# ska-telescope/ska-sdp-idg-bench

Hardware: AMD Instinct MI355X
Metric: Mvisibilities/s (gridder & degridder) at 1/2/4/8 GPUs; % HBM roofline (higher is better)
Workload: dtype f32 phase/accumulate, f16x2-split MFMA operands

## Files before the change

### ska-sdp-idg-bench_amd/csrc/hip/kernels/gridder_mi355x.hip.cpp

```cpp
#include <hip/hip_runtime.h>

#include <cstdlib>
#include <string>

#include "../util.hpp"
#include "device.hpp"
#include "fft.hpp"
#include "lib-hip.hpp"
#include "mfma.hpp"

#ifndef IDG_GRID_PT
#define IDG_GRID_PT 4
#endif
#ifndef IDG_GRID_WAVES
#define IDG_GRID_WAVES 4
#endif
#ifndef IDG_GRID_WAVES_GENERAL
#define IDG_GRID_WAVES_GENERAL 4
#endif
#ifndef IDG_GRID_FUSED_GENERAL
#define IDG_GRID_FUSED_GENERAL 1
#endif
#ifndef IDG_GRID_BSCALE
#define IDG_GRID_BSCALE 12
#endif
#ifndef IDG_GRID_NT_FILL
#define IDG_GRID_NT_FILL 0
#endif
#ifndef IDG_GRID_NW
#define IDG_GRID_NW 8
#endif

namespace idg_mi355x {

namespace {

__device__ __forceinline__ void mac4(float *a, const float4 &va,
                                     const float4 &vb, float cs, float sn) {
  a[0] = fma_(va.x, cs, a[0]); a[0] = fma_(-va.y, sn, a[0]);
  a[1] = fma_(va.x, sn, a[1]); a[1] = fma_(va.y, cs, a[1]);
  a[2] = fma_(va.z, cs, a[2]); a[2] = fma_(-va.w, sn, a[2]);
  a[3] = fma_(va.z, sn, a[3]); a[3] = fma_(va.w, cs, a[3]);
  a[4] = fma_(vb.x, cs, a[4]); a[4] = fma_(-vb.y, sn, a[4]);
  a[5] = fma_(vb.x, sn, a[5]); a[5] = fma_(vb.y, cs, a[5]);
  a[6] = fma_(vb.z, cs, a[6]); a[6] = fma_(-vb.w, sn, a[6]);
  a[7] = fma_(vb.z, sn, a[7]); a[7] = fma_(vb.w, cs, a[7]);
}

template <int NP, int CB>
__device__ __forceinline__ void timestep_general(
    const float (&l)[NP], const float (&m)[NP], const float (&n)[NP],
    const float (&poff)[NP], float (&acc)[NP][8],
    const idg::UVWCoordinate<float> c, const float4 *__restrict__ vrow,
    const float *__restrict__ wavenumbers, int C) {
  float pidx[NP];
#pragma unroll
  for (int i = 0; i < NP; ++i)
    pidx[i] = fma_(c.w, n[i], fma_(c.u, l[i], c.v * m[i]));
  for (int cb = 0; cb < C; cb += CB) {
    const int ce = min(cb + CB, C);
    const float k0 = wavenumbers[cb];
    float A[NP], R[NP];
#pragma unroll
    for (int i = 0; i < NP; ++i) {
      A[i] = fma_(-pidx[i], k0, poff[i]);
      R[i] = revolutions(A[i]);
    }
    float k = k0;
    float4 va = vrow[2 * cb], vb = vrow[2 * cb + 1];
    for (int ch = cb; ch < ce; ++ch) {
      const int nx = min(ch + 1, C - 1);
      const float kn = wavenumbers[nx];
      const float4 van = vrow[2 * nx], vbn = vrow[2 * nx + 1];
#pragma unroll
      for (int i = 0; i < NP; ++i) {
        const float ph = fma_(-pidx[i], k, poff[i]);
        const float r = fma_(ph - A[i], kInv2PiHi, R[i]);
        float sn, cs;
        sincos_rev(r, &sn, &cs);
        mac4(acc[i], va, vb, cs, sn);
      }
      k = kn;
      va = van;
      vb = vbn;
    }
  }
}

template <int NB, int CB>
__device__ __forceinline__ void timestep_mirror(
    const float (&l)[2 * NB], const float (&m)[2 * NB],
    const float (&poff)[2 * NB], float (&acc)[2 * NB][8],
    const idg::UVWCoordinate<float> c, const float4 *__restrict__ vrow,
    const float *__restrict__ wavenumbers, int C) {
  float pidx[NB];
#pragma unroll
  for (int i = 0; i < NB; ++i) pidx[i] = fma_(c.u, l[i], c.v * m[i]);
  for (int cb = 0; cb < C; cb += CB) {
    const int ce = min(cb + CB, C);
    const float k0 = wavenumbers[cb];
    float A[NB], R[NB];
#pragma unroll
    for (int i = 0; i < NB; ++i) {
      A[i] = fma_(-pidx[i], k0, poff[i]);
      R[i] = revolutions(A[i]);
    }
    float k = k0;
    float4 va = vrow[2 * cb], vb = vrow[2 * cb + 1];
    for (int ch = cb; ch < ce; ++ch) {
      const int nx = min(ch + 1, C - 1);
      const float kn = wavenumbers[nx];
      const float4 van = vrow[2 * nx], vbn = vrow[2 * nx + 1];
#pragma unroll
      for (int i = 0; i < NB; ++i) {
        const float ph = fma_(-pidx[i], k, poff[i]);
        const float r = fma_(ph - A[i], kInv2PiHi, R[i]);
        float sn, cs;
        sincos_rev(r, &sn, &cs);
        mac4(acc[i], va, vb, cs, sn);
        mac4(acc[NB + i], va, vb, cs, -sn);
      }
      k = kn;
      va = van;
      vb = vbn;
    }
  }
}

__device__ __forceinline__ void pixel_out(const float (&a)[8], int p, int S,
                                          const SubgridSetup &g,
                                          int nr_stations,
                                          const float *__restrict__ spheroidal,
                                          const float2 *__restrict__ aterms,
                                          float2 (&o)[4]) {
  const int y = p / S, x = p - (p / S) * S;
  idg::cfloat pix[4], a1[4], a2[4];
  for (int q = 0; q < 4; ++q) pix[q] = {a[2 * q], a[2 * q + 1]};
  load_jones(aterm_ptr(aterms, nr_stations, S, g.aterm_index, g.station1, y,
                       x), a1);
  load_jones(aterm_ptr(aterms, nr_stations, S, g.aterm_index, g.station2, y,
                       x), a2);
  idg::apply_aterm_gridder(pix, a1, a2);
  const float sph = spheroidal[p];
#pragma unroll
  for (int q = 0; q < 4; ++q) o[q] = make_float2(pix[q].re * sph, pix[q].im * sph);
}

__device__ __forceinline__ void store_pixel(
    const float (&a)[8], int p, int S, int npix, const SubgridSetup &g,
    int nr_stations, const float *__restrict__ spheroidal,
    const float2 *__restrict__ aterms, float2 *__restrict__ out) {
  float2 o[4];
  pixel_out(a, p, S, g, nr_stations, spheroidal, aterms, o);
#pragma unroll
  for (int q = 0; q < 4; ++q) out[static_cast<size_t>(q) * npix + p] = o[q];
}

template <bool W_TERMS = true>
__device__ __forceinline__ void pixel_geometry(int p, int S, float image_size,
                                               const SubgridSetup &g,
                                               float &l, float &m, float &n,
                                               float &poff) {
  const int y = p / S, x = p - (p / S) * S;
  l = idg::compute_l(x, S, image_size);
  m = idg::compute_m(y, S, image_size);
  if constexpr (W_TERMS) {
    n = idg::compute_n(l, m);
    poff = fma_(g.w_offset, n, fma_(g.u_offset, l, g.v_offset * m));
  } else {
    n = 0.0f;
    poff = fma_(g.u_offset, l, g.v_offset * m);
  }
}


#ifndef IDG_GRID_KSBUF
#define IDG_GRID_KSBUF 32
#endif
constexpr int kKsBuf = IDG_GRID_KSBUF;

template <int AT, int NW>
struct MfmaLds {
  static constexpr int kObufFloats = NW * 16 * AT * 16;
  static constexpr int kBbufWords = kKsBuf * 64 * 8;
  static constexpr int kUvwOff =
      kObufFloats > kBbufWords ? kObufFloats : kBbufWords;
  static constexpr int kRedOff = kUvwOff + 4 * 4 * kKsBuf;
  static constexpr int kSlotOff = kRedOff + 8;
  static constexpr int kSinkOff = kSlotOff + 2;
  static constexpr int kWords = kSinkOff + 64;
  static constexpr int kGeoOff = kWords;
  static constexpr int kWordsGeo = kGeoOff + 64 + 2 * 1024;
};
template <int S_CT, int NW, int AT>
constexpr int general_lds_words() {
  return S_CT == 32 ? MfmaLds<AT, NW>::kWordsGeo : MfmaLds<AT, NW>::kWords;
}

__device__ __forceinline__ void l2_prefetch_dma(const void *src,
                                                const void *lds_dst) {
  const unsigned m0 = __builtin_amdgcn_readfirstlane(static_cast<unsigned>(
      reinterpret_cast<size_t>((const __attribute__((address_space(3))) void *)
                                   lds_dst)));
  unsigned saved;
  asm volatile(
      "s_mov_b32 %0, m0\n\ts_mov_b32 m0, %2\n\ts_nop 0\n\t"
      "global_load_lds_dword %1, off\n\ts_mov_b32 m0, %0"
      : "=&s"(saved)
      : "v"(src), "s"(m0)
      : "memory");
}

template <int S_CT, int PT, int CB, int NW, bool MIRROR, bool FFT = false,
          int PREC = kPrecTail, bool PRESCAN = false, bool OPAQUE_TID = !MIRROR>
__device__ __forceinline__ void grid_mfma(
    const SubgridSetup &g, int S, int npix, float image_size, int C,
    int nr_stations, const idg::UVWCoordinate<float> *__restrict__ uvw,
    const float *__restrict__ wavenumbers,
    const float2 *__restrict__ visibilities,
    const float *__restrict__ spheroidal, const float2 *__restrict__ aterms,
    float2 *__restrict__ out, unsigned *lds, float vmax_pre = 0.0f,
    int pass_lo = 0, int pass_hi = 1 << 30) {
  static_assert(CB % 4 == 0, "anchor blocks hold whole channel quads");
  int tid = threadIdx.x;
  if constexpr (OPAQUE_TID) asm volatile("" : "+v"(tid));
  const int lane = tid & 63, wave = tid >> 6;
  const int grp = lane >> 4, col = lane & 15;
  const int half = MIRROR ? npix / 2 : npix;
  constexpr bool kFused = !MIRROR && IDG_GRID_FUSED_GENERAL;
  constexpr bool kTailAlt = (PREC & kPrecTailAlt) != 0;
  constexpr bool kTailAll = (PREC & kPrecTail) != 0 && !kTailAlt;
  constexpr int AT = kFused ? PT : 2 * PT;
  using Lds = MfmaLds<AT, NW>;
  constexpr bool kGeoLds = kFused && S_CT == 32;
  float *geo = reinterpret_cast<float *>(lds + Lds::kGeoOff);
  const int nt = g.nr_timesteps;
  const int nchq = (C + 3) / 4;
  const int nquads = (nt + 3) / 4;
  const int quads_per_fill = nchq <= kKsBuf ? kKsBuf / nchq : 1;
  const int cq_per_fill = nchq <= kKsBuf ? nchq : kKsBuf;
  unsigned *slots = lds + Lds::kSlotOff;

  float vmax = vmax_pre;
  if (tid < 2) slots[tid] = 0u;
  if constexpr (!PRESCAN) {
    vmax = 0.0f;
    const float4 *v4 = reinterpret_cast<const float4 *>(
        visibilities + g.time_offset * C * 4);
    const int n4 = min(4 * quads_per_fill, nt) * C * 2;
    for (int i = tid; i < n4; i += NW * 64) {
      const float4 q = v4[i];
      vmax = fmaxf(vmax, fmaxf(fmaxf(fabsf(q.x), fabsf(q.y)),
                               fmaxf(fabsf(q.z), fabsf(q.w))));
    }
    for (int off = 32; off > 0; off >>= 1)
      vmax = fmaxf(vmax, __shfl_xor(vmax, off));
    float *red = reinterpret_cast<float *>(lds + Lds::kRedOff);
    if (lane == 0) red[wave] = vmax;
    __syncthreads();
#pragma unroll
    for (int w = 0; w < NW; ++w) vmax = fmaxf(vmax, red[w]);
  }
  constexpr int kBS = IDG_GRID_BSCALE;
  static_assert(kBS >= 0 && kBS <= 14, "a fill may reach 2^15 before it re-splits");
  int e = 0;
  bool have_scale = vmax > 0.0f && vmax <= 3.0e38f;
  if (have_scale) frexpf(vmax, &e);
  float scale = ldexpf(1.0f, kBS - e);
  int fidx = 0;

  const float2 *__restrict__ vsub = visibilities + g.time_offset * C * 4;

  uint4 *bbuf = reinterpret_cast<uint4 *>(lds);
  float *obuf = reinterpret_cast<float *>(lds);
  float4 *tuvw = reinterpret_cast<float4 *>(lds + Lds::kUvwOff);

  constexpr int kPass = NW * 16 * PT;
  for (int gbase = pass_lo; gbase < min(half, pass_hi); gbase += kPass) {
    static_assert(PT % 2 == 0, "phases are packed over tile pairs");
    constexpr int PH = PT / 2;
    floatx2 L2[PH], M2[PH], N2[PH], PG2[PH];
    if constexpr (kGeoLds) {
      static_assert(PT == 8 && NW == 8, "one S = 32 pass: 1,024 pixels");
      for (int p = tid; p < 1024; p += NW * 64) {
        float l, m, n, pg;
        pixel_geometry<true>(p, 32, image_size, g, l, m, n, pg);
        geo[64 + p] = n;
        geo[64 + 1024 + p] = pg;
        if (p < 32) geo[p] = l;
        if (p % 32 == 0) geo[32 + p / 32] = m;
      }
    } else {
#pragma unroll
      for (int i = 0; i < PT; ++i) {
        const int b = min(gbase + (wave * PT + i) * 16 + col, half - 1);
        float l, m, n, pg;
        pixel_geometry<!MIRROR>(b, S, image_size, g, l, m, n, pg);
        L2[i / 2][i % 2] = l;
        M2[i / 2][i % 2] = m;
        N2[i / 2][i % 2] = n;
        PG2[i / 2][i % 2] = pg;
      }
    }
    constexpr int PY = kFused ? 1 : PT;
    floatx4 accx[PT], accy[PY];
#pragma unroll
    for (int i = 0; i < PT; ++i) accx[i] = floatx4{0.0f, 0.0f, 0.0f, 0.0f};
#pragma unroll
    for (int i = 0; i < PY; ++i) accy[i] = floatx4{0.0f, 0.0f, 0.0f, 0.0f};

    constexpr bool kFlush = (PREC & kPrecFlush) != 0;
    static_assert(!kFlush || S_CT == 32,
                  "the master fills the S = 32 output slot in one pass");
    bool flushed = false;
    auto master = [&](int t) {
      return reinterpret_cast<float4 *>(out) +
             ((wave * AT + t) * 32 + grp * 8 + (col & 7));
    };
    auto flush_tile = [&](floatx4 &a, int t, float unsc) {
      const float a0 = a[0], a1 = a[1], a2 = a[2], a3 = a[3];
      const float v0 = (a0 + row_ror8(a0)) * unsc;
      const float v1 = (a1 + row_ror8(a1)) * unsc;
      const float v2 = (a2 + row_ror8(a2)) * unsc;
      const float v3 = (a3 + row_ror8(a3)) * unsc;
      if (col < 8) {
        float4 m = make_float4(0.0f, 0.0f, 0.0f, 0.0f);
        if (flushed) m = *master(t);
        *master(t) = make_float4(m.x + v0, m.y + v1, m.z + v2, m.w + v3);
      }
      a = floatx4{0.0f, 0.0f, 0.0f, 0.0f};
    };

    for (int q0 = 0; q0 < nquads; q0 += quads_per_fill) {
      const int nq = min(quads_per_fill, nquads - q0);
      for (int j0 = 0; j0 < nchq; j0 += cq_per_fill, ++fidx) {
        const int nj = min(cq_per_fill, nchq - j0);
        for (;;) {
        __syncthreads();
        if (tid == 0) slots[(fidx + 1) & 1] = 0u;
        {
          const int bpol = (col & 7) >> 1;
          const int w_c = 2 * bpol + (col & 1);
          const int w_s = 2 * bpol + 1 - (col & 1);
          const float sc_s = (col & 1) ? scale : -scale;
          const float bpart = (col & 8) ? -1.0f : 0.0f;
          const float *vsubf = reinterpret_cast<const float *>(vsub);
          const int nks = nq * nj;
          const bool full = (q0 + nq) * 4 <= nt && 4 * (j0 + nj) <= C;
          const int wv = __builtin_amdgcn_readfirstlane(wave);
          const unsigned off_c = (grp * C * 8 + w_c) * 4u;
          const unsigned off_s = (grp * C * 8 + w_s) * 4u;
          int qq = wv / nj, jj = wv - (wv / nj) * nj;
          float lmax = 0.0f;
#ifdef IDG_DEBUG_SKIPFILL
          for (int ks = fidx > 0 ? nks : wv; ks < nks; ks += NW) {
#else
          for (int ks = wv; ks < nks; ks += NW) {
#endif
            const int t = (q0 + qq) * 4 + grp;
            const int c0 = 4 * (j0 + jj);
            float bc[4], bs[4];
            if (full) {
              const char *blk = reinterpret_cast<const char *>(
                  vsubf + ((q0 + qq) * 4 * C + c0) * 8);
#pragma unroll
              for (int u = 0; u < 4; ++u) {
#if IDG_GRID_NT_FILL
                const __amdgpu_buffer_rsrc_t rsrc =
                    __builtin_amdgcn_make_buffer_rsrc(
                        const_cast<char *>(blk), static_cast<short>(0),
                        0x7ffffff0, 0x00020000);
                const float rc = __builtin_bit_cast(
                    float, __builtin_amdgcn_raw_buffer_load_b32(
                               rsrc, static_cast<int>(off_c), 32 * u, 2));
                const float rs = __builtin_bit_cast(
                    float, __builtin_amdgcn_raw_buffer_load_b32(
                               rsrc, static_cast<int>(off_s), 32 * u, 2));
#else
                const float rc =
                    *reinterpret_cast<const float *>(blk + off_c + 32 * u);
                const float rs =
                    *reinterpret_cast<const float *>(blk + off_s + 32 * u);
#endif
                lmax = fmaxf(lmax, fmaxf(fabsf(rc), fabsf(rs)));
                bc[u] = rc * scale;
                bs[u] = rs * sc_s;
              }
            } else {
#pragma unroll
              for (int u = 0; u < 4; ++u) {
                const bool ok = t < nt && c0 + u < C;
                const int it = ok ? t * C + c0 + u : 0;
                const float rc = ok ? vsubf[it * 8 + w_c] : 0.0f;
                const float rs = ok ? vsubf[it * 8 + w_s] : 0.0f;
                lmax = fmaxf(lmax, fmaxf(fabsf(rc), fabsf(rs)));
                bc[u] = rc * scale;
                bs[u] = rs * sc_s;
              }
            }
            jj += NW;
            while (jj >= nj) {
              jj -= nj;
              ++qq;
            }
            const unsigned xc = split_part(bc[0], bc[1], bpart);
            const unsigned yc = split_part(bc[2], bc[3], bpart);
            const unsigned xs = split_part(bs[0], bs[1], bpart);
            const unsigned ys = split_part(bs[2], bs[3], bpart);
            bbuf[(ks * 64 + lane) * 2] = make_uint4(xc, xc, yc, yc);
            bbuf[(ks * 64 + lane) * 2 + 1] = make_uint4(xs, xs, ys, ys);
          }
          {
            unsigned v = __float_as_uint(lmax);
            v = max(v, (unsigned)__builtin_amdgcn_update_dpp(0, (int)v, 0xB1, 0xF, 0xF, false));
            v = max(v, (unsigned)__builtin_amdgcn_update_dpp(0, (int)v, 0x4E, 0xF, 0xF, false));
            v = max(v, (unsigned)__builtin_amdgcn_update_dpp(0, (int)v, 0x124, 0xF, 0xF, false));
            v = max(v, (unsigned)__builtin_amdgcn_update_dpp(0, (int)v, 0x128, 0xF, 0xF, false));
            const unsigned wmax =
                max(max(__builtin_amdgcn_readlane(v, 0), __builtin_amdgcn_readlane(v, 16)),
                    max(__builtin_amdgcn_readlane(v, 32), __builtin_amdgcn_readlane(v, 48)));
            if (lane == 0) atomicMax(&slots[fidx & 1], wmax);
          }
          for (int i = tid; i < nq * 4; i += NW * 64) {
            const idg::UVWCoordinate<float> c =
                uvw[g.time_offset + min(q0 * 4 + i, nt - 1)];
            tuvw[i] = make_float4(c.u, c.v, c.w, 0.0f);
          }
        }
        __syncthreads();
        const float fm = __uint_as_float(
            __builtin_amdgcn_readfirstlane(slots[fidx & 1]));
        if (!(fm > 0.0f && fm <= 3.0e38f)) break;
        int em;
        frexpf(fm, &em);
        if (have_scale ? em <= e + 15 - kBS : em == e) {
          have_scale = true;
          break;
        }
        if (have_scale) {
          const float r = ldexpf(1.0f, e - em);
#pragma unroll
          for (int i = 0; i < PT; ++i) accx[i] *= r;
#pragma unroll
          for (int i = 0; i < PY; ++i) accy[i] *= r;
        }
        e = em;
        scale = ldexpf(1.0f, kBS - e);
        have_scale = true;
        }
        {
          int q0n = q0, j0n = j0 + cq_per_fill;
          if (j0n >= nchq) {
            j0n = 0;
            q0n = q0 + quads_per_fill;
          }
          if (q0n < nquads) {
            const int rows = min(4 * (q0n + quads_per_fill), nt) - 4 * q0n;
            const int lpr = (min(cq_per_fill, nchq - j0n) * 128 + 127) / 128;
            const char *vb = reinterpret_cast<const char *>(vsub);
            for (int ln = tid; ln < rows * lpr; ln += NW * 64) {
              const int row = ln / lpr, cl = ln - (ln / lpr) * lpr;
              l2_prefetch_dma(
                  vb + (static_cast<size_t>(4 * q0n + row) * C + 4 * j0n) * 32 +
                      cl * 128,
                  lds + Lds::kSinkOff);
            }
          }
        }
        for (int jb = 0; jb < nj; jb += CB / 4) {
          const int je = min(jb + CB / 4, nj);
          const float ka = wavenumbers[4 * (j0 + jb)];
          float kb[CB];
#pragma unroll
          for (int v = 0; v < CB; ++v)
            kb[v] = wavenumbers[min(4 * (j0 + jb) + v, C - 1)];
          for (int qq = 0; qq < nq; ++qq) {
            const float4 c4 = tuvw[qq * 4 + grp];
            const idg::UVWCoordinate<float> c = {c4.x, c4.y, c4.z};
            const floatx2 cu = {c.u, c.u}, cv = {c.v, c.v};
            const floatx2 ih = {kInv2PiHi, kInv2PiHi};
            if constexpr (kFused) {
#pragma unroll
              for (int h = 0; h < PH; ++h) {
                if constexpr (kGeoLds) {
                  const int b0 = (wave * PT + 2 * h) * 16 + col;
                  L2[h] = floatx2{geo[col], geo[col + 16]};
                  const float mh = geo[32 + wave * (PT / 2) + h];
                  M2[h] = floatx2{mh, mh};
                  N2[h] = floatx2{geo[64 + b0], geo[64 + b0 + 16]};
                  PG2[h] = floatx2{geo[64 + 1024 + b0], geo[64 + 1024 + b0 + 16]};
                }
                floatx2 pidx = __builtin_elementwise_fma(cu, L2[h], cv * M2[h]);
                pidx = __builtin_elementwise_fma(floatx2{c.w, c.w}, N2[h], pidx);
                const floatx2 np = -pidx;
                const floatx2 a =
                    __builtin_elementwise_fma(np, floatx2{ka, ka}, PG2[h]);
                const floatx2 t = a * ih;
                const floatx2 nm = {-__builtin_rintf(t.x), -__builtin_rintf(t.y)};
                floatx2 cr = {0.0f, 0.0f};
                if constexpr (kTailAll) cr = tail_k_rev(np, ka);
                if constexpr (kTailAlt)
                  cr = tail_k_rev(np, 4.0f * ka);
#pragma unroll
                for (int u = 0; u < CB / 4; ++u) {
                  const int jj = jb + u;
                  if (jj >= je) break;
                  const int ks = qq * nj + jj;
                  const uint4 bx = bbuf[(ks * 64 + lane) * 2];
                  const uint4 by = bbuf[(ks * 64 + lane) * 2 + 1];
                  const half8 bfx = pack4(bx.x, bx.y, bx.z, bx.w);
                  const half8 bfy = pack4(by.x, by.y, by.z, by.w);
                  float snx[4], csx[4], sny[4], csy[4];
#pragma unroll
                  for (int j = 0; j < 4; ++j) {
                    const float kj = kb[4 * u + j];
                    const floatx2 ph =
                        __builtin_elementwise_fma(np, floatx2{kj, kj}, PG2[h]);
                    floatx2 r = __builtin_elementwise_fma(ph, ih, nm);
                    if constexpr (kTailAll) r = r + cr;
                    if constexpr (kTailAlt)
                      if (j == 0) r = r + cr;
                    sincos_rev(r.x, &snx[j], &csx[j]);
                    sincos_rev(r.y, &sny[j], &csy[j]);
                  }
                  half8 ac, as, ac1, as1;
                  split_oct(csx[0], csx[1], csx[2], csx[3], snx[0], snx[1],
                            snx[2], snx[3], &ac, &as);
                  split_oct(csy[0], csy[1], csy[2], csy[3], sny[0], sny[1],
                            sny[2], sny[3], &ac1, &as1);
                  accx[2 * h] = mfma16(ac, bfx, accx[2 * h]);
                  accx[2 * h + 1] = mfma16(ac1, bfx, accx[2 * h + 1]);
                  accx[2 * h] = mfma16(as, bfy, accx[2 * h]);
                  accx[2 * h + 1] = mfma16(as1, bfy, accx[2 * h + 1]);
                  IDG_KSTEP_FENCE();
                }
              }
              continue;
            }
            floatx2 NP[PH], NM[PH], CR[PH];
#pragma unroll
            for (int h = 0; h < PH; ++h) {
              floatx2 pidx = __builtin_elementwise_fma(cu, L2[h], cv * M2[h]);
              if constexpr (!MIRROR)
                pidx = __builtin_elementwise_fma(floatx2{c.w, c.w}, N2[h],
                                                 pidx);
              NP[h] = -pidx;
              const floatx2 a =
                  __builtin_elementwise_fma(NP[h], floatx2{ka, ka}, PG2[h]);
              const floatx2 t = a * ih;
              NM[h] = floatx2{-__builtin_rintf(t.x), -__builtin_rintf(t.y)};
              if constexpr (kTailAll)
                CR[h] = tail_k_rev(NP[h], ka);
              if constexpr (kTailAlt)
                CR[h] = tail_k_rev(NP[h], 4.0f * ka);
            }
#pragma unroll
            for (int u = 0; u < CB / 4; ++u) {
              const int jj = jb + u;
              if (jj >= je) break;
              const int ks = qq * nj + jj;
              const uint4 bx = bbuf[(ks * 64 + lane) * 2];
              const uint4 by = bbuf[(ks * 64 + lane) * 2 + 1];
              const half8 bfx = pack4(bx.x, bx.y, bx.z, bx.w);
              const half8 bfy = pack4(by.x, by.y, by.z, by.w);
#pragma unroll
              for (int h = 0; h < PH; ++h) {
                float snx[4], csx[4], sny[4], csy[4];
#pragma unroll
                for (int j = 0; j < 4; ++j) {
                  const float kj = kb[4 * u + j];
                  const floatx2 ph =
                      __builtin_elementwise_fma(NP[h], floatx2{kj, kj}, PG2[h]);
                  floatx2 r = __builtin_elementwise_fma(ph, ih, NM[h]);
                  if constexpr (kTailAll) r = r + CR[h];
                  if constexpr (kTailAlt)
                    if (j == 0) r = r + CR[h];
                  sincos_rev(r.x, &snx[j], &csx[j]);
                  sincos_rev(r.y, &sny[j], &csy[j]);
                }
                half8 ac, as;
                split_oct(csx[0], csx[1], csx[2], csx[3], snx[0], snx[1],
                          snx[2], snx[3], &ac, &as);
                accx[2 * h] = mfma16(ac, bfx, accx[2 * h]);
                accy[2 * h] = mfma16(as, bfy, accy[2 * h]);
                split_oct(csy[0], csy[1], csy[2], csy[3], sny[0], sny[1],
                          sny[2], sny[3], &ac, &as);
                accx[2 * h + 1] = mfma16(ac, bfx, accx[2 * h + 1]);
                accy[2 * h + 1] = mfma16(as, bfy, accy[2 * h + 1]);
              }
              IDG_KSTEP_FENCE();
            }
          }
        }
        if constexpr (kFlush) {
          const bool last =
              j0 + cq_per_fill >= nchq && q0 + quads_per_fill >= nquads;
          if (!last && (fidx + 1) % kFlushFills == 0) {
            const float unsc = ldexpf(1.0f, e - kBS);
#pragma unroll
            for (int i = 0; i < PT; ++i) flush_tile(accx[i], i, unsc);
            if constexpr (!kFused) {
#pragma unroll
              for (int i = 0; i < PY; ++i) flush_tile(accy[i], PT + i, unsc);
            }
            flushed = true;
          }
        }
      }
    }
    if constexpr (kFlush) {
      if (flushed && col < 8) {
        const float sc = ldexpf(1.0f, kBS - e);
#pragma unroll
        for (int i = 0; i < PT; ++i) {
          const float4 m = *master(i);
          accx[i] += floatx4{m.x, m.y, m.z, m.w} * sc;
        }
        if constexpr (!kFused) {
#pragma unroll
          for (int i = 0; i < PY; ++i) {
            const float4 m = *master(PT + i);
            accy[i] += floatx4{m.x, m.y, m.z, m.w} * sc;
          }
        }
      }
    }

    const float unscale = ldexpf(1.0f, e - kBS);
    __syncthreads();
#pragma unroll
    for (int i = 0; i < PT; ++i)
#pragma unroll
      for (int r = 0; r < 4; ++r) {
        const int lp = (wave * PT + i) * 16 + grp * 4 + r;
        obuf[lp * 16 + col] = accx[i][r];
        if constexpr (!kFused) obuf[(kPass + lp) * 16 + col] = accy[i][r];
      }
    __syncthreads();
    static_assert(!FFT || (S_CT == 32 && kPass >= (MIRROR ? 512 : 1024)),
                  "the FFT epilogue takes a whole S = 32 subgrid in one pass");
    constexpr int kIt = FFT ? kPass / (NW * 64) : 1;
    float2 keep[kIt][MIRROR ? 2 : 1][4];
    auto emit = [&](const float (&a)[8], int p, int it, int slot) {
      if constexpr (FFT)
        pixel_out(a, p, S, g, nr_stations, spheroidal, aterms, keep[it][slot]);
      else
        store_pixel(a, p, S, npix, g, nr_stations, spheroidal, aterms, out);
    };
    auto body = [&](int q, int it) {
      const int b = gbase + q;
      if (b >= half) return;
      const float4 *xr = reinterpret_cast<const float4 *>(obuf + q * 16);
      const float4 xh0 = xr[0], xh1 = xr[1], xl0 = xr[2], xl1 = xr[3];
      const float x[8] = {xh0.x + xl0.x, xh0.y + xl0.y, xh0.z + xl0.z,
                          xh0.w + xl0.w, xh1.x + xl1.x, xh1.y + xl1.y,
                          xh1.z + xl1.z, xh1.w + xl1.w};
      float y[8] = {0.0f, 0.0f, 0.0f, 0.0f, 0.0f, 0.0f, 0.0f, 0.0f};
      if constexpr (!kFused) {
        const float4 *yr =
            reinterpret_cast<const float4 *>(obuf + (kPass + q) * 16);
        const float4 yh0 = yr[0], yh1 = yr[1], yl0 = yr[2], yl1 = yr[3];
        const float yv[8] = {yh0.x + yl0.x, yh0.y + yl0.y, yh0.z + yl0.z,
                             yh0.w + yl0.w, yh1.x + yl1.x, yh1.y + yl1.y,
                             yh1.z + yl1.z, yh1.w + yl1.w};
#pragma unroll
        for (int j = 0; j < 8; ++j) y[j] = yv[j];
      }
      float l, m, n, poff;
      pixel_geometry<!MIRROR>(b, S, image_size, g, l, m, n, poff);
      float tc, ts;
      phase_tail(poff, &tc, &ts);
      float ab[8];
#pragma unroll
      for (int j = 0; j < 8; ++j)
        ab[j] = (kFused ? x[j] : x[j] + y[j]) * unscale;
      rotate4(ab, tc, ts);
      emit(ab, b, it, 0);
      if constexpr (MIRROR) {
        float am[8];
#pragma unroll
        for (int j = 0; j < 8; ++j) am[j] = (x[j] - y[j]) * unscale;
        rotate4(am, tc, -ts);
        emit(am, npix - 1 - b, it, 1);
      }
    };
    if constexpr (FFT) {
#pragma unroll
      for (int it = 0; it < kIt; ++it) body(tid + it * NW * 64, it);
      constexpr int N = 32, RS = N + 1;
      float2 *planes = reinterpret_cast<float2 *>(lds);
      __syncthreads();
#pragma unroll
      for (int it = 0; it < kIt; ++it) {
        const int b = tid + it * NW * 64;
        if (b >= half) continue;
#pragma unroll
        for (int slot = 0; slot < (MIRROR ? 2 : 1); ++slot) {
          const int p = slot ? npix - 1 - b : b;
          const int row = p / N, col = p % N;
#pragma unroll
          for (int pol = 0; pol < 4; ++pol)
            planes[pol * N * RS + row * RS + col] = keep[it][slot][pol];
        }
      }
      __syncthreads();
      float2 tw[N / 2];
#pragma unroll
      for (int k = 0; k < N / 2; ++k) tw[k] = unit_phasor(k, N, 1.0f);
      float2 f[N];
      fft2_planes_lds<N>(planes, tid, 4 * N, tw, f);
      if (tid < 4 * N) {
        const int pp = tid / N, qq = tid % N;
#pragma unroll
        for (int i = 0; i < N; ++i)
          out[static_cast<size_t>(pp) * npix + bit_reverse<N>(i) * N + qq] =
              f[i];
      }
    } else {
      for (int q = tid; q < kPass; q += NW * 64) body(q, 0);
    }
    __syncthreads();
  }
}

template <int NW>
__device__ __forceinline__ bool prologue_scan(
    const SubgridSetup &g, int C,
    const idg::UVWCoordinate<float> *__restrict__ uvw,
    const float2 *__restrict__ visibilities, float *red) {
  const int tid = threadIdx.x;
  bool w_nonzero = false;
  for (int t = tid; t < g.nr_timesteps; t += NW * 64)
    w_nonzero |= uvw[g.time_offset + t].w != 0.0f;
  const int nchq = (C + 3) / 4;
  const int quads_per_fill = nchq <= kKsBuf ? kKsBuf / nchq : 1;
  const float4 *v4 = reinterpret_cast<const float4 *>(
      visibilities + g.time_offset * C * 4);
  const int n4 = min(4 * quads_per_fill, g.nr_timesteps) * C * 2;
  float vmax = 0.0f;
  for (int i = tid; i < n4; i += NW * 64) {
    const float4 q = v4[i];
    vmax = fmaxf(vmax, fmaxf(fmaxf(fabsf(q.x), fabsf(q.y)),
                             fmaxf(fabsf(q.z), fabsf(q.w))));
  }
  for (int off = 32; off > 0; off >>= 1)
    vmax = fmaxf(vmax, __shfl_xor(vmax, off));
  if ((tid & 63) == 0) red[tid >> 6] = vmax;
  return w_nonzero;
}

template <int NW>
__device__ __forceinline__ float prologue_max(const float *red) {
  float vmax = red[0];
#pragma unroll
  for (int w = 1; w < NW; ++w) vmax = fmaxf(vmax, red[w]);
  return vmax;
}

}

#if defined(IDG_WG_TIMELINE) && IDG_WG_TIMELINE
__device__ WgStamp idg_debug_timeline_gridder[kTimelineMax];
#endif

template <int S_CT, int PPT, int CB, int MODE, int PT, bool FFT = false,
          int PREC = kPrecTail>
__global__ void __launch_bounds__(MODE == 1 ? 64 * IDG_GRID_NW : kBlock,
                                  IDG_GRID_WAVES)
    kernel_gridder_mi355x(const int grid_size, int subgrid_size,
                          float image_size, float w_step_in_lambda,
                          int nr_channels, int nr_stations,
                          const idg::UVWCoordinate<float> *__restrict__ uvw,
                          const float *__restrict__ wavenumbers,
                          const float2 *__restrict__ visibilities,
                          const float *__restrict__ spheroidal,
                          const float2 *__restrict__ aterms,
                          const idg::Metadata *__restrict__ metadata,
                          float2 *__restrict__ subgrids) {
  static_assert(PPT % 2 == 0, "PPT must be even (pixel pairs)");
  constexpr int NB = PPT / 2;
  const int S = S_CT > 0 ? S_CT : subgrid_size;
  const int npix = S * S;
  const int s = xcd_subgrid(blockIdx.x, gridDim.x);
  const int tid = threadIdx.x;
  const SubgridSetup g = setup_subgrid(metadata, s, grid_size, S, image_size,
                                       w_step_in_lambda);
  const int C = nr_channels;
  float2 *out = subgrids + static_cast<size_t>(s) * 4 * npix;

  if constexpr (MODE == 1) {
    constexpr int NW = IDG_GRID_NW;
    __shared__ unsigned lds[general_lds_words<S_CT, NW, 2 * PT>()];
#if defined(IDG_WG_TIMELINE) && IDG_WG_TIMELINE
    timeline_start(idg_debug_timeline_gridder);
#endif
    float *red = reinterpret_cast<float *>(lds + MfmaLds<2 * PT, NW>::kRedOff);
    const bool mirror =
        __syncthreads_or(prologue_scan<NW>(g, C, uvw, visibilities, red)) ==
            0 &&
        S % 2 == 0 && g.w_offset == 0.0f;
    const float vmax = prologue_max<NW>(red);
    if (mirror)
      grid_mfma<S_CT, PT, CB, NW, true, FFT, PREC, true>(
          g, S, npix, image_size, C, nr_stations, uvw, wavenumbers,
          visibilities, spheroidal, aterms, out, lds, vmax);
    else
      grid_mfma<S_CT, IDG_GRID_FUSED_GENERAL ? 2 * PT : PT, CB, NW, false,
                FFT, PREC, true>(g, S, npix, image_size, C, nr_stations, uvw,
                                 wavenumbers, visibilities, spheroidal, aterms,
                                 out, lds, vmax);
#if defined(IDG_WG_TIMELINE) && IDG_WG_TIMELINE
    timeline_end(idg_debug_timeline_gridder);
#endif
    return;
  }

  bool w_nonzero = false;
  for (int t = tid; t < g.nr_timesteps; t += blockDim.x)
    w_nonzero |= uvw[g.time_offset + t].w != 0.0f;
  const bool mirror = __syncthreads_or(w_nonzero) == 0 && S % 2 == 0 &&
                      g.w_offset == 0.0f;

  if (mirror) {
    const int half = npix / 2;
    for (int tile = 0; tile < half; tile += kBlock * NB) {
      float l[PPT], m[PPT], n[PPT], poff[PPT], acc[PPT][8];
#pragma unroll
      for (int i = 0; i < NB; ++i) {
        const int b = min(tile + i * kBlock + tid, half - 1);
        pixel_geometry(b, S, image_size, g, l[i], m[i], n[i], poff[i]);
        pixel_geometry(npix - 1 - b, S, image_size, g, l[NB + i], m[NB + i],
                       n[NB + i], poff[NB + i]);
      }
#pragma unroll
      for (int i = 0; i < PPT; ++i)
#pragma unroll
        for (int j = 0; j < 8; ++j) acc[i][j] = 0.0f;

      for (int t = 0; t < g.nr_timesteps; ++t) {
        const long long row = g.time_offset + t;
        const idg::UVWCoordinate<float> c = uvw[row];
        const float4 *vrow =
            reinterpret_cast<const float4 *>(visibilities + row * C * 4);
        timestep_mirror<NB, CB>(l, m, poff, acc, c, vrow, wavenumbers, C);
      }
#pragma unroll
      for (int i = 0; i < NB; ++i) {
        const int b = tile + i * kBlock + tid;
        if (b < half) {
          store_pixel(acc[i], b, S, npix, g, nr_stations, spheroidal, aterms,
                      out);
          store_pixel(acc[NB + i], npix - 1 - b, S, npix, g, nr_stations,
                      spheroidal, aterms, out);
        }
      }
    }
    return;
  }

  for (int tile = 0; tile < npix; tile += kBlock * PPT) {
    float l[PPT], m[PPT], n[PPT], poff[PPT], acc[PPT][8];
#pragma unroll
    for (int i = 0; i < PPT; ++i) {
      const int p = min(tile + i * kBlock + tid, npix - 1);
      pixel_geometry(p, S, image_size, g, l[i], m[i], n[i], poff[i]);
#pragma unroll
      for (int j = 0; j < 8; ++j) acc[i][j] = 0.0f;
    }
    for (int t = 0; t < g.nr_timesteps; ++t) {
      const long long row = g.time_offset + t;
      const idg::UVWCoordinate<float> c = uvw[row];
      const float4 *vrow =
          reinterpret_cast<const float4 *>(visibilities + row * C * 4);
      timestep_general<PPT, CB>(l, m, n, poff, acc, c, vrow, wavenumbers, C);
    }
#pragma unroll
    for (int i = 0; i < PPT; ++i) {
      const int p = tile + i * kBlock + tid;
      if (p < npix)
        store_pixel(acc[i], p, S, npix, g, nr_stations, spheroidal, aterms,
                    out);
    }
  }
}

template <int S_CT, int CB, int PT, bool FFT = false, int PREC = kPrecTail,
          int SPLIT = 1>
__global__ void __launch_bounds__(64 * IDG_GRID_NW, IDG_GRID_WAVES)
    kernel_gridder_mirror_mi355x(
        const int grid_size, int subgrid_size, float image_size,
        float w_step_in_lambda, int nr_channels, int nr_stations,
        const idg::UVWCoordinate<float> *__restrict__ uvw,
        const float *__restrict__ wavenumbers,
        const float2 *__restrict__ visibilities,
        const float *__restrict__ spheroidal,
        const float2 *__restrict__ aterms,
        const idg::Metadata *__restrict__ metadata,
        float2 *__restrict__ subgrids, int *__restrict__ queue) {
  constexpr int NW = IDG_GRID_NW;
  __shared__ unsigned lds[MfmaLds<2 * PT, NW>::kWords];
  const int S = S_CT > 0 ? S_CT : subgrid_size;
  const int npix = S * S;
  const int wg = xcd_subgrid(blockIdx.x, gridDim.x);
  const int s = SPLIT > 1 ? wg / SPLIT : wg;
  const int q = SPLIT > 1 ? wg % SPLIT : 0;
  const int tid = threadIdx.x;
  const SubgridSetup g = setup_subgrid(metadata, s, grid_size, S, image_size,
                                       w_step_in_lambda);
  float *red = reinterpret_cast<float *>(lds + MfmaLds<2 * PT, NW>::kRedOff);
  const bool mirror =
      __syncthreads_or(prologue_scan<NW>(g, nr_channels, uvw, visibilities,
                                         red)) == 0 &&
      S % 2 == 0 && g.w_offset == 0.0f;
  if (!mirror) {
    if constexpr (SPLIT > 1) {
      if (tid == 0 && q == 0)
        queue_push(queue, gridDim.x / SPLIT, s, s % kQueueShards);
    } else {
      if (tid == 0) queue_push(queue, gridDim.x, s);
    }
    return;
  }
  constexpr int kPass = NW * 16 * PT;
  static_assert(SPLIT == 1 || (S_CT > 0 && SPLIT * kPass >= S_CT * S_CT / 2 &&
                               (SPLIT - 1) * kPass < S_CT * S_CT / 2),
                "mirror_split(S) does not match the pass size");
  grid_mfma<S_CT, PT, CB, NW, true, FFT, PREC, true>(
      g, S, npix, image_size, nr_channels, nr_stations, uvw, wavenumbers,
      visibilities, spheroidal, aterms,
      subgrids + static_cast<size_t>(s) * 4 * npix, lds,
      prologue_max<NW>(red), SPLIT > 1 ? q * kPass : 0,
      SPLIT > 1 ? (q + 1) * kPass : 1 << 30);
}

template <int S_CT, int CB, int PT, bool FFT = false, int PREC = kPrecTail>
__global__ void __launch_bounds__(64 * IDG_GRID_NW, IDG_GRID_WAVES)
    kernel_gridder_mirror_persist_mi355x(
        const int grid_size, int subgrid_size, float image_size,
        float w_step_in_lambda, int nr_channels, int nr_stations,
        const idg::UVWCoordinate<float> *__restrict__ uvw,
        const float *__restrict__ wavenumbers,
        const float2 *__restrict__ visibilities,
        const float *__restrict__ spheroidal,
        const float2 *__restrict__ aterms,
        const idg::Metadata *__restrict__ metadata,
        float2 *__restrict__ subgrids, int *__restrict__ queue,
        int nr_subgrids) {
  constexpr int NW = IDG_GRID_NW;
  __shared__ unsigned lds[MfmaLds<2 * PT, NW>::kWords];
  __shared__ int take;
  const int S = S_CT > 0 ? S_CT : subgrid_size;
  const int npix = S * S;
  const int tid = threadIdx.x;
  if (tid == 0) take = atomicAdd(queue + kQueueMirror, 1);
  __syncthreads();
  int i = __builtin_amdgcn_readfirstlane(take);
  while (i < nr_subgrids) {
    __syncthreads();
    if (tid == 0) take = atomicAdd(queue + kQueueMirror, 1);
    const int s = i;
    const SubgridSetup g = setup_subgrid(metadata, s, grid_size, S,
                                         image_size, w_step_in_lambda);
    float *red = reinterpret_cast<float *>(lds + MfmaLds<2 * PT, NW>::kRedOff);
    const bool mirror =
        __syncthreads_or(prologue_scan<NW>(g, nr_channels, uvw, visibilities,
                                           red)) == 0 &&
        S % 2 == 0 && g.w_offset == 0.0f;
    if (!mirror) {
      if (tid == 0) queue_push(queue, nr_subgrids, s, s % kQueueShards);
    } else {
      grid_mfma<S_CT, PT, CB, NW, true, FFT, PREC, true, true>(
          g, S, npix, image_size, nr_channels, nr_stations, uvw, wavenumbers,
          visibilities, spheroidal, aterms,
          subgrids + static_cast<size_t>(s) * 4 * npix, lds,
          prologue_max<NW>(red), 0, 1 << 30);
    }
    __syncthreads();
    i = __builtin_amdgcn_readfirstlane(take);
  }
  if (tid == 0 && atomicAdd(queue + kQueueMirrorExit, 1) ==
                      static_cast<int>(gridDim.x) - 1) {
    queue[kQueueMirror] = 0;
    queue[kQueueMirrorExit] = 0;
  }
}

template <int S_CT, int CB, int PT, bool FFT = false, int PREC = kPrecTail>
__global__ void __launch_bounds__(64 * IDG_GRID_NW, IDG_GRID_WAVES_GENERAL)
    kernel_gridder_general_mi355x(
        const int grid_size, int subgrid_size, float image_size,
        float w_step_in_lambda, int nr_channels, int nr_stations,
        const idg::UVWCoordinate<float> *__restrict__ uvw,
        const float *__restrict__ wavenumbers,
        const float2 *__restrict__ visibilities,
        const float *__restrict__ spheroidal,
        const float2 *__restrict__ aterms,
        const idg::Metadata *__restrict__ metadata,
        float2 *__restrict__ subgrids, int *__restrict__ queue,
        int nr_subgrids, int all) {
  constexpr int NW = IDG_GRID_NW;
  __shared__ unsigned lds[general_lds_words<S_CT, NW, 2 * PT>()];
  const int S = S_CT > 0 ? S_CT : subgrid_size;
  const int npix = S * S;
  const int tid = threadIdx.x;
  const QueueView qv = queue_view(queue, nr_subgrids);
  const int count = all ? nr_subgrids : qv.count();
  if (count == 0) return;
  if (tid == 0)
    lds[0] = static_cast<unsigned>(atomicAdd(queue + kQueueNext, 1));
  __syncthreads();
  int i = static_cast<int>(__builtin_amdgcn_readfirstlane(lds[0]));
  __syncthreads();
  while (i < count) {
    int next = 0;
    if (tid == 0) next = atomicAdd(queue + kQueueNext, 1);
    const int s = all ? i : qv.at(i);
    const SubgridSetup g = setup_subgrid(metadata, s, grid_size, S,
                                         image_size, w_step_in_lambda);
    grid_mfma<S_CT, IDG_GRID_FUSED_GENERAL ? 2 * PT : PT, CB, NW, false, FFT,
              PREC>(
        g, S, npix, image_size, nr_channels, nr_stations, uvw, wavenumbers,
        visibilities, spheroidal, aterms,
        subgrids + static_cast<size_t>(s) * 4 * npix, lds);
    if (tid == 0) lds[0] = static_cast<unsigned>(next);
    __syncthreads();
    i = static_cast<int>(__builtin_amdgcn_readfirstlane(lds[0]));
    __syncthreads();
  }
  if (tid == 0) queue_retire(queue);
}

struct GridderSet {
  const void *combined, *mirror, *general;
};
#ifndef IDG_GRID_SPLIT64
#define IDG_GRID_SPLIT64 1
#endif
#ifndef IDG_GRID_PERSIST
#define IDG_GRID_PERSIST 0
#endif
constexpr int mirror_split(int S) {
  return S == 64 && IDG_GRID_SPLIT64 ? 4 : 1;
}
template <int S_, bool FFT_, int PREC_>
const void *mirror_kernel() {
  if constexpr (IDG_GRID_PERSIST && S_ == 32)
    return reinterpret_cast<const void *>(
        &kernel_gridder_mirror_persist_mi355x<S_, 16, IDG_GRID_PT, FFT_,
                                              PREC_>);
  else
    return reinterpret_cast<const void *>(
        &kernel_gridder_mirror_mi355x<S_, 16, IDG_GRID_PT, FFT_, PREC_,
                                      mirror_split(S_)>);
}
template <int S_, int PPT_, bool FFT_, int PREC_>
GridderSet gridder_set() {
  return {reinterpret_cast<const void *>(
              &kernel_gridder_mi355x<S_, PPT_, 16, 1, IDG_GRID_PT, FFT_, PREC_>),
          mirror_kernel<S_, FFT_, PREC_>(),
          reinterpret_cast<const void *>(
              &kernel_gridder_general_mi355x<S_, 16, IDG_GRID_PT, FFT_, PREC_>)};
}
template <int S_, int PPT_, bool FFT_>
GridderSet gridder_set_for(int prec) {
  if (prec & kPrecTailAlt) prec &= ~kPrecTail;
  if constexpr (S_ == 32) {
    switch (prec) {
      case 0: return gridder_set<S_, PPT_, FFT_, 0>();
      case kPrecTail | kPrecFlush:
        return gridder_set<S_, PPT_, FFT_, kPrecTail | kPrecFlush>();
      case kPrecFlush: return gridder_set<S_, PPT_, FFT_, kPrecFlush>();
      case kPrecTailAlt: return gridder_set<S_, PPT_, FFT_, kPrecTailAlt>();
      case kPrecTailAlt | kPrecFlush:
        return gridder_set<S_, PPT_, FFT_, kPrecTailAlt | kPrecFlush>();
      default: return gridder_set<S_, PPT_, FFT_, kPrecTail>();
    }
  } else {
    if (prec & kPrecTailAlt) return gridder_set<S_, PPT_, FFT_, kPrecTailAlt>();
    return (prec & kPrecTail) ? gridder_set<S_, PPT_, FFT_, kPrecTail>()
                              : gridder_set<S_, PPT_, FFT_, 0>();
  }
}
#define IDG_GRIDDER_VALU(S_, PPT_)                                        \
  reinterpret_cast<const void *>(                                         \
      &kernel_gridder_mi355x<S_, PPT_, 16, 0, IDG_GRID_PT>)

#ifndef IDG_GRID_SPLIT
#define IDG_GRID_SPLIT 1
#endif

static int gridder_impl() {
  const char *v = std::getenv("IDG_GRIDDER_IMPL");
  if (v && std::string(v) == "sequential") return 2;
  return (v && std::string(v) == "valu") ? 0 : 1;
}

KernelChoice select_gridder(const Problem &p) {
  KernelChoice k;
  k.grid = p.nr_subgrids;
  if (gridder_impl() == 2) {
    k.func = sequential_gridder(p.subgrid_size);
    k.block = sequential_block();
    k.name = p.subgrid_size == 32   ? "gridder_sequential_mi355x_s32"
             : p.subgrid_size == 64 ? "gridder_sequential_mi355x_s64"
                                    : "gridder_sequential_mi355x_generic";
    return k;
  }
  const bool mfma = gridder_impl() == 1;
  k.block = mfma ? 64 * IDG_GRID_NW : kBlock;
  k.prec = precision_for(Direction::kGridder, p);
  if (k.prec & kPrecTailAlt) k.prec &= ~kPrecTail;
  if (p.subgrid_size != 32) k.prec &= ~kPrecFlush;
  if (!mfma) k.prec = 0;
  const char *fenv = std::getenv("IDG_GRID_FFT");
  const bool fft_epilogue = p.fft_out && mfma && p.subgrid_size == 32 &&
                            !(fenv != nullptr && fenv[0] == '0');
  GridderSet set{};
  switch (p.subgrid_size) {
    case 32:
      set = fft_epilogue ? gridder_set_for<32, 4, true>(k.prec)
                         : gridder_set_for<32, 4, false>(k.prec);
      k.name = fft_epilogue ? "gridder_fft_mi355x_s32"
                            : (mfma ? "gridder_mi355x_s32"
                                    : "gridder_mi355x_s32_valu");
      k.fft_in_kernel = fft_epilogue;
      if (!mfma) set.combined = IDG_GRIDDER_VALU(32, 4);
      break;
    case 64:
      set = gridder_set_for<64, 4, false>(k.prec);
      k.name = mfma ? "gridder_mi355x_s64" : "gridder_mi355x_s64_valu";
      if (!mfma) set.combined = IDG_GRIDDER_VALU(64, 4);
      break;
    default:
      set = gridder_set_for<0, 2, false>(k.prec);
      k.name = mfma ? "gridder_mi355x_generic" : "gridder_mi355x_generic_valu";
      if (p.subgrid_size % 2 != 0) set.mirror = nullptr;
      if (!mfma) set.combined = IDG_GRIDDER_VALU(0, 2);
      break;
  }
  k.func = set.combined;
  if (mfma && IDG_GRID_SPLIT && two_kernel_form(p.nr_subgrids)) {
    if (set.mirror)
      k.parts[0] = {set.mirror, k.block, KernelChoice::kMirror,
                    p.subgrid_size == 64 ? mirror_split(64)
                    : IDG_GRID_PERSIST && p.subgrid_size == 32 ? 0
                                                               : 1};
    k.parts[1] = {set.general, k.block, KernelChoice::kGeneral};
    k.all_general = {k.func, k.block, KernelChoice::kPlain};
  }
  return k;
}

}

namespace hip {

void p_run_gridder() {
  idg_mi355x::Problem p;
  p.subgrid_size = static_cast<int>(get_env_var("SUBGRID_SIZE", 32));
  p.nr_channels = static_cast<int>(get_env_var("NR_CHANNELS", 16));
  const idg_mi355x::KernelChoice k = idg_mi355x::select_gridder(p);
  p_run_gridder_(k.func, "gridder_mi355x", k.block);
}

void c_run_gridder(
    int nr_subgrids, int grid_size, int subgrid_size, float image_size,
    float w_step_in_lambda, int nr_channels, int nr_stations,
    idg::Array2D<idg::UVWCoordinate<float>> &uvw,
    idg::Array1D<float> &wavenumbers,
    idg::Array3D<idg::Visibility<std::complex<float>>> &visibilities,
    idg::Array2D<float> &spheroidal,
    idg::Array4D<idg::Matrix2x2<std::complex<float>>> &aterms,
    idg::Array1D<idg::Metadata> &metadata,
    idg::Array4D<std::complex<float>> &subgrids) {
  c_run_gridder_(nr_subgrids, grid_size, subgrid_size, image_size,
                 w_step_in_lambda, nr_channels, nr_stations, uvw, wavenumbers,
                 visibilities, spheroidal, aterms, metadata, subgrids, nullptr,
                 0);
}

}

#if defined(IDG_WG_TIMELINE) && IDG_WG_TIMELINE
extern "C" int idg_debug_timeline_gridder_copy(void *host, int n) {
  return hipMemcpyFromSymbol(
      host, HIP_SYMBOL(idg_mi355x::idg_debug_timeline_gridder),
      sizeof(WgStamp) * std::min(n, kTimelineMax));
}
#endif
```

Baseline: 3294.

## Store one B fragment per step in mirror gridder and derive sine part by rotation

In the mirror path, the LDS B buffer now holds only the cosine-weighted fragment per k-step. The sine-side result is rebuilt afterwards by swapping and negating the real and imaginary parts of the accumulated output. This halves LDS footprint per step, so each fill can cover twice as many k-steps, and the flush period is rescaled to match. Fill loads are batched to a configurable depth so several global loads are in flight before LDS writes. The risks are numerical-layout correctness of the rotation trick and higher register pressure from the deeper fill.

Result: faster. 3350, median of 6 (+1.7%).

```diff
diff --git a/ska-sdp-idg-bench_amd/csrc/hip/kernels/gridder_mi355x.hip.cpp b/ska-sdp-idg-bench_amd/csrc/hip/kernels/gridder_mi355x.hip.cpp
--- a/ska-sdp-idg-bench_amd/csrc/hip/kernels/gridder_mi355x.hip.cpp
+++ b/ska-sdp-idg-bench_amd/csrc/hip/kernels/gridder_mi355x.hip.cpp
@@ -178,11 +178,22 @@
 #define IDG_GRID_KSBUF 32
 #endif
 constexpr int kKsBuf = IDG_GRID_KSBUF;
+#ifndef IDG_GRID_KSBUF_MIRROR
+#define IDG_GRID_KSBUF_MIRROR (2 * IDG_GRID_KSBUF)
+#endif
+constexpr int kKsBufMirror = IDG_GRID_KSBUF_MIRROR;
+#ifndef IDG_GRID_FILL_DEPTH
+#define IDG_GRID_FILL_DEPTH 2
+#endif
+constexpr int mirror_fill_depth(int S_CT, bool combined) {
+  return combined && S_CT != 32 ? 1 : IDG_GRID_FILL_DEPTH;
+}
 
 template <int AT, int NW>
 struct MfmaLds {
   static constexpr int kObufFloats = NW * 16 * AT * 16;
   static constexpr int kBbufWords = kKsBuf * 64 * 8;
+  static_assert(kKsBufMirror * 64 * 4 <= kBbufWords, "one buffer, two layouts");
   static constexpr int kUvwOff =
       kObufFloats > kBbufWords ? kObufFloats : kBbufWords;
   static constexpr int kRedOff = kUvwOff + 4 * 4 * kKsBuf;
@@ -212,7 +223,8 @@
 }
 
 template <int S_CT, int PT, int CB, int NW, bool MIRROR, bool FFT = false,
-          int PREC = kPrecTail, bool PRESCAN = false, bool OPAQUE_TID = !MIRROR>
+          int PREC = kPrecTail, bool PRESCAN = false, bool OPAQUE_TID = !MIRROR,
+          int FILL_D = IDG_GRID_FILL_DEPTH>
 __device__ __forceinline__ void grid_mfma(
     const SubgridSetup &g, int S, int npix, float image_size, int C,
     int nr_stations, const idg::UVWCoordinate<float> *__restrict__ uvw,
@@ -237,8 +249,10 @@
   const int nt = g.nr_timesteps;
   const int nchq = (C + 3) / 4;
   const int nquads = (nt + 3) / 4;
-  const int quads_per_fill = nchq <= kKsBuf ? kKsBuf / nchq : 1;
-  const int cq_per_fill = nchq <= kKsBuf ? nchq : kKsBuf;
+  constexpr bool kOneFrag = MIRROR && S_CT != 0;
+  constexpr int KS = kOneFrag ? kKsBufMirror : kKsBuf;
+  const int quads_per_fill = nchq <= KS ? min(KS / nchq, kKsBuf) : 1;
+  const int cq_per_fill = nchq <= KS ? nchq : KS;
   unsigned *slots = lds + Lds::kSlotOff;
 
   float vmax = vmax_pre;
@@ -353,10 +367,70 @@
           int qq = wv / nj, jj = wv - (wv / nj) * nj;
           float lmax = 0.0f;
 #ifdef IDG_DEBUG_SKIPFILL
-          for (int ks = fidx > 0 ? nks : wv; ks < nks; ks += NW) {
+          const int ks_first = fidx > 0 ? nks : wv;
 #else
-          for (int ks = wv; ks < nks; ks += NW) {
-#endif
+          const int ks_first = wv;
+#endif
+          if constexpr (kOneFrag) {
+            auto load4 = [&](int q_, int j_, float (&b)[4]) {
+              const int c0 = 4 * (j0 + j_);
+              if (full) {
+                const char *blk = reinterpret_cast<const char *>(
+                    vsubf + ((q0 + q_) * 4 * C + c0) * 8);
+#pragma unroll
+                for (int u = 0; u < 4; ++u) {
+#if IDG_GRID_NT_FILL
+                  const __amdgpu_buffer_rsrc_t rsrc =
+                      __builtin_amdgcn_make_buffer_rsrc(
+                          const_cast<char *>(blk), static_cast<short>(0),
+                          0x7ffffff0, 0x00020000);
+                  b[u] = __builtin_bit_cast(
+                      float, __builtin_amdgcn_raw_buffer_load_b32(
+                                 rsrc, static_cast<int>(off_c), 32 * u, 2));
+#else
+                  b[u] = *reinterpret_cast<const float *>(blk + off_c + 32 * u);
+#endif
+                }
+              } else {
+                const int t = (q0 + q_) * 4 + grp;
+#pragma unroll
+                for (int u = 0; u < 4; ++u) {
+                  const bool ok = t < nt && c0 + u < C;
+                  b[u] = ok ? vsubf[(t * C + c0 + u) * 8 + w_c] : 0.0f;
+                }
+              }
+            };
+            auto put = [&](int ks, const float (&b)[4]) {
+              lmax = fmaxf(lmax, fmaxf(fmaxf(fabsf(b[0]), fabsf(b[1])),
+                                       fmaxf(fabsf(b[2]), fabsf(b[3]))));
+              const unsigned xc =
+                  split_part(b[0] * scale, b[1] * scale, bpart);
+              const unsigned yc =
+                  split_part(b[2] * scale, b[3] * scale, bpart);
+              bbuf[ks * 64 + lane] = make_uint4(xc, xc, yc, yc);
+            };
+            auto advance = [&]() {
+              jj += NW;
+              while (jj >= nj) {
+                jj -= nj;
+                ++qq;
+              }
+            };
+            constexpr int D = FILL_D;
+            for (int ks = ks_first; ks < nks; ks += D * NW) {
+              float b[D][4];
+#pragma unroll
+              for (int d = 0; d < D; ++d)
+                if (ks + d * NW < nks) {
+                  load4(qq, jj, b[d]);
+                  advance();
+                }
+#pragma unroll
+              for (int d = 0; d < D; ++d)
+                if (ks + d * NW < nks) put(ks + d * NW, b[d]);
+            }
+          } else {
+          for (int ks = ks_first; ks < nks; ks += NW) {
             const int t = (q0 + qq) * 4 + grp;
             const int c0 = 4 * (j0 + jj);
             float bc[4], bs[4];
@@ -409,6 +483,7 @@
             const unsigned ys = split_part(bs[2], bs[3], bpart);
             bbuf[(ks * 64 + lane) * 2] = make_uint4(xc, xc, yc, yc);
             bbuf[(ks * 64 + lane) * 2 + 1] = make_uint4(xs, xs, ys, ys);
+          }
           }
           {
             unsigned v = __float_as_uint(lmax);
@@ -559,8 +634,9 @@
               const int jj = jb + u;
               if (jj >= je) break;
               const int ks = qq * nj + jj;
-              const uint4 bx = bbuf[(ks * 64 + lane) * 2];
-              const uint4 by = bbuf[(ks * 64 + lane) * 2 + 1];
+              const int fr = ks * 64 + lane;
+              const uint4 bx = bbuf[kOneFrag ? fr : 2 * fr];
+              const uint4 by = kOneFrag ? bx : bbuf[2 * fr + 1];
               const half8 bfx = pack4(bx.x, bx.y, bx.z, bx.w);
               const half8 bfy = pack4(by.x, by.y, by.z, by.w);
 #pragma unroll
@@ -593,9 +669,12 @@
           }
         }
         if constexpr (kFlush) {
+          constexpr int kFlushEvery = kFlushFills * kKsBuf / KS;
+          static_assert(kFlushEvery * KS == kFlushFills * kKsBuf,
+                        "the flush period is a whole number of fills");
           const bool last =
               j0 + cq_per_fill >= nchq && q0 + quads_per_fill >= nquads;
-          if (!last && (fidx + 1) % kFlushFills == 0) {
+          if (!last && (fidx + 1) % kFlushEvery == 0) {
             const float unsc = ldexpf(1.0f, e - kBS);
 #pragma unroll
             for (int i = 0; i < PT; ++i) flush_tile(accx[i], i, unsc);
@@ -663,8 +742,16 @@
         const float yv[8] = {yh0.x + yl0.x, yh0.y + yl0.y, yh0.z + yl0.z,
                              yh0.w + yl0.w, yh1.x + yl1.x, yh1.y + yl1.y,
                              yh1.z + yl1.z, yh1.w + yl1.w};
-#pragma unroll
-        for (int j = 0; j < 8; ++j) y[j] = yv[j];
+        if constexpr (kOneFrag) {
+#pragma unroll
+          for (int k = 0; k < 4; ++k) {
+            y[2 * k] = -yv[2 * k + 1];
+            y[2 * k + 1] = yv[2 * k];
+          }
+        } else {
+#pragma unroll
+          for (int j = 0; j < 8; ++j) y[j] = yv[j];
+        }
       }
       float l, m, n, poff;
       pixel_geometry<!MIRROR>(b, S, image_size, g, l, m, n, poff);
@@ -801,7 +888,8 @@
         S % 2 == 0 && g.w_offset == 0.0f;
     const float vmax = prologue_max<NW>(red);
     if (mirror)
-      grid_mfma<S_CT, PT, CB, NW, true, FFT, PREC, true>(
+      grid_mfma<S_CT, PT, CB, NW, true, FFT, PREC, true, false,
+                mirror_fill_depth(S_CT, true)>(
           g, S, npix, image_size, C, nr_stations, uvw, wavenumbers,
           visibilities, spheroidal, aterms, out, lds, vmax);
     else
@@ -925,7 +1013,8 @@
   static_assert(SPLIT == 1 || (S_CT > 0 && SPLIT * kPass >= S_CT * S_CT / 2 &&
                                (SPLIT - 1) * kPass < S_CT * S_CT / 2),
                 "mirror_split(S) does not match the pass size");
-  grid_mfma<S_CT, PT, CB, NW, true, FFT, PREC, true>(
+  grid_mfma<S_CT, PT, CB, NW, true, FFT, PREC, true, false,
+            mirror_fill_depth(S_CT, false)>(
       g, S, npix, image_size, nr_channels, nr_stations, uvw, wavenumbers,
       visibilities, spheroidal, aterms,
       subgrids + static_cast<size_t>(s) * 4 * npix, lds,
```
